# voithru/voice-activity-detection

Hardware: AMD Instinct MI355X
Metric: audio frames/sec (whole node) (higher is better)
Workload: dtype f32 (bf16x6 split operands, f32 accumulate)

## Files before the change

voice_activity_detection_amd/csrc/savad_kernels_f32s.h:

```cpp
#pragma once
#include "savad_kernels_bf16.h"
#include <type_traits>

namespace savad {
#ifdef SAVAD_TIMING
__device__ long long g_savad_wg[1024][4];
#endif
namespace fs {

using bf::bf16x8;
using bf::u32x4;
using bf::ldfrag;
using bf::stfrag;
using bf::FRAG_BYTES;
using bf::slot_row;
using bf::AttnState;
using bf::attn_state_init;
using bf::online_softmax_shifted;

constexpr int SLOT_BYTES = 2 * BLK3_BYTES;
constexpr int NRING3 = 3;
constexpr int ROW_LDS_BYTES = NRING3 * SLOT_BYTES + 9 * D * 4;

struct Tri {
    bf16x8 h, m, l;
};

__device__ __forceinline__ void split1(float a, __bf16& h, __bf16& m, __bf16& l) {
    h = (__bf16)a;
    if (SAVAD_ABLATE & 128) {
        m = l = h;
        return;
    }
    const float r1 = a - (float)h;
    m = (__bf16)r1;
    const float r2 = r1 - (float)m;
    l = (__bf16)r2;
}
__device__ __forceinline__ Tri split8(const float (&v)[8]) {
    Tri t;
#pragma unroll
    for (int e = 0; e < 8; ++e) {
        __bf16 h, m, l;
        split1(v[e], h, m, l);
        t.h[e] = h;
        t.m[e] = m;
        t.l[e] = l;
    }
    return t;
}
__device__ __forceinline__ Tri split_half(const f32x16& v, int j) {
    float t[8];
#pragma unroll
    for (int e = 0; e < 8; ++e) t[e] = v[8 * j + e];
    return split8(t);
}
__device__ __forceinline__ void split_row(const f32x4 (&xg)[16], Tri (&xp)[8]) {
#pragma unroll
    for (int ks = 0; ks < 8; ++ks) {
        float t[8];
#pragma unroll
        for (int e = 0; e < 8; ++e) t[e] = xg[2 * ks + (e >> 2)][e & 3];
        xp[ks] = split8(t);
    }
}
__device__ __forceinline__ Tri ldtri(const char* p ) {
    return Tri{ldfrag(p), ldfrag(p + FRAG_BYTES), ldfrag(p + 2 * FRAG_BYTES)};
}
__device__ __forceinline__ void sttri(char* p, const Tri& t) {
    stfrag(p, t.h);
    stfrag(p + FRAG_BYTES, t.m);
    stfrag(p + 2 * FRAG_BYTES, t.l);
}
__device__ __forceinline__ Tri zero_tri() {
    const bf16x8 z = __builtin_bit_cast(bf16x8, u32x4{0u, 0u, 0u, 0u});
    return Tri{z, z, z};
}

#define SAVAD_MF(a, b, c) __builtin_amdgcn_mfma_f32_32x32x16_bf16((a), (b), (c), 0, 0, 0)
template <bool SWAP>
__device__ __forceinline__ void mfma6x2_lo(f32x16& acc0, f32x16& acc1, const Tri& a0, const Tri& a1, const Tri& b) {
#define SAVAD_MF2(pa, pb)                                                           \
    acc0 = SWAP ? SAVAD_MF(b.pb, a0.pa, acc0) : SAVAD_MF(a0.pa, b.pb, acc0);        \
    acc1 = SWAP ? SAVAD_MF(b.pb, a1.pa, acc1) : SAVAD_MF(a1.pa, b.pb, acc1);
    SAVAD_MF2(h, l) SAVAD_MF2(l, h) SAVAD_MF2(m, m)
}
template <bool SWAP>
__device__ __forceinline__ void mfma6x2_hi(f32x16& acc0, f32x16& acc1, const Tri& a0, const Tri& a1, const Tri& b) {
    SAVAD_MF2(h, m) SAVAD_MF2(m, h) SAVAD_MF2(h, h)
#undef SAVAD_MF2
}
template <bool SWAP>
__device__ __forceinline__ void mfma6x2(f32x16& acc0, f32x16& acc1, const Tri& a0, const Tri& a1, const Tri& b) {
    mfma6x2_lo<SWAP>(acc0, acc1, a0, a1, b);
    mfma6x2_hi<SWAP>(acc0, acc1, a0, a1, b);
}

__device__ __forceinline__ void load_hblock32(f32x16 (&x)[4], const float* hb, int lane) {
#pragma unroll
    for (int nb = 0; nb < 4; ++nb)
#pragma unroll
        for (int g = 0; g < 4; ++g) {
            const f32x4 t = ld4(hb + ((nb * 4 + g) * 64 + lane) * 4);
#pragma unroll
            for (int s = 0; s < 4; ++s) x[nb][4 * g + s] += t[s];
        }
}
__device__ __forceinline__ void request_hblock32(f32x4 (&hr)[16], const float* hb , int lane) {
#define SAVAD_H_LD(i)                                                                                                          \
    asm volatile("global_load_dwordx4 %0, %1, %2 offset:%3" : "+v"(hr[i]) : "v"((unsigned)lane * 16u + 4096u * ((i) / 4)), "s"(hb), \
                 "n"(((i) % 4) * 1024) : "memory")
    SAVAD_H_LD(0); SAVAD_H_LD(1); SAVAD_H_LD(2); SAVAD_H_LD(3); SAVAD_H_LD(4); SAVAD_H_LD(5); SAVAD_H_LD(6); SAVAD_H_LD(7);
    SAVAD_H_LD(8); SAVAD_H_LD(9); SAVAD_H_LD(10); SAVAD_H_LD(11); SAVAD_H_LD(12); SAVAD_H_LD(13); SAVAD_H_LD(14); SAVAD_H_LD(15);
#undef SAVAD_H_LD
}
__device__ __forceinline__ void landed_hblock32(f32x4 (&hr)[16]) {
    asm volatile("" : "+v"(hr[0]), "+v"(hr[1]), "+v"(hr[2]), "+v"(hr[3]), "+v"(hr[4]), "+v"(hr[5]), "+v"(hr[6]), "+v"(hr[7]), "+v"(hr[8]),
                 "+v"(hr[9]), "+v"(hr[10]), "+v"(hr[11]), "+v"(hr[12]), "+v"(hr[13]), "+v"(hr[14]), "+v"(hr[15]));
}
__device__ __forceinline__ void store_hblock32(float* hb, const f32x16 (&x)[4], int lane) {
#pragma unroll
    for (int nb = 0; nb < 4; ++nb)
#pragma unroll
        for (int g = 0; g < 4; ++g) {
            f32x4 t;
#pragma unroll
            for (int s = 0; s < 4; ++s) t[s] = x[nb][4 * g + s];
            st4(hb + ((nb * 4 + g) * 64 + lane) * 4, t);
        }
}

#ifndef SAVAD_PIECE_FENCE
#define SAVAD_PIECE_FENCE 0x6
#endif
struct DmaJob {
    const char* src;
    unsigned ldsb;
};
struct Ring3 {
    static constexpr int PER = 12;
    char* base;
    int w, lane;
    unsigned voff[3];

    __device__ __forceinline__ Ring3(char* smem, int w_, int lane_) : base(smem), w(w_), lane(lane_) {
#pragma unroll
        for (int g = 0; g < 3; ++g) voff[g] = (unsigned)lane_ * 16u + 4096u * g;
    }
    __device__ __forceinline__ char* slot(int t) const { return base + (t % NRING3) * SLOT_BYTES; }
    __device__ __forceinline__ DmaJob job(int t, const char* seg0, const char* seg1) const {
        const unsigned slot0 = __builtin_amdgcn_readfirstlane((unsigned)(size_t)slot(t));
        return DmaJob{((w >> 1) ? seg1 : seg0) + (size_t)(w & 1) * (BLK3_BYTES / 2), slot0 + (unsigned)w * (BLK3_BYTES / 2)};
    }
    template <int I>
    __device__ __forceinline__ void piece(const DmaJob& j) const {
        if (SAVAD_ABLATE & 1) return;
        __builtin_amdgcn_sched_barrier(SAVAD_PIECE_FENCE);
        piece_raw<I>(j);
        __builtin_amdgcn_sched_barrier(SAVAD_PIECE_FENCE);
    }
    template <int I>
    __device__ __forceinline__ void piece_raw(const DmaJob& j) const {
        asm volatile(
            "s_add_u32 m0, %2, %3\n\t"
            "s_nop 0\n\t"
            "global_load_lds_dwordx4 %0, %1 offset:%4"
            :
            : "v"(voff[I / 4]), "s"(j.src), "s"(j.ldsb), "n"((I / 4) * 4096), "n"((I % 4) * 1024)
            : "memory", "scc");
    }
    __device__ __forceinline__ void issue_all(const DmaJob& j) const {
        if (SAVAD_ABLATE & 1) return;
        piece_raw<0>(j); piece_raw<1>(j); piece_raw<2>(j); piece_raw<3>(j); piece_raw<4>(j); piece_raw<5>(j);
        piece_raw<6>(j); piece_raw<7>(j); piece_raw<8>(j); piece_raw<9>(j); piece_raw<10>(j); piece_raw<11>(j);
    }
    template <int NEWER>
    __device__ __forceinline__ void acquire() const {
        if (SAVAD_ABLATE & 2) return;
        __builtin_amdgcn_s_waitcnt(bf::Ring<4>::vmcnt_imm(NEWER * PER));
        asm volatile("" ::: "memory");
        __syncthreads();
    }
};

struct NoMid {
    template <int KS>
    __device__ __forceinline__ void operator()(std::integral_constant<int, KS>) const {}
};
template <bool SWAP, bool DMA, class Mid = NoMid>
__device__ __forceinline__ void gemm_slot(f32x16& acc0, f32x16& acc1, const char* slot, const Tri (&xp)[8], const Ring3& ring,
                                          const DmaJob& job, const Mid& mid = Mid{}) {
    if (SAVAD_ABLATE & 8) {
#pragma unroll
        for (int ks = 0; ks < 8; ++ks) mfma6x2<SWAP>(acc0, acc1, xp[7 - ks], xp[ks ^ 1], xp[ks]);
        return;
    }
    const unsigned a = (unsigned)(size_t)slot + (unsigned)ring.lane * 16u;
    u32x4 f[2][6];
#define SAVAD_G_LD(ks, i) asm volatile("ds_read_b128 %0, %1 offset:%2" : "=v"(f[(ks) & 1][i]) : "v"(a), "n"(((i) / 3) * BLK3_BYTES + (ks) * TFRAG_BYTES + ((i) % 3) * FRAG_BYTES))
#define SAVAD_G_LD6(ks) SAVAD_G_LD(ks, 0); SAVAD_G_LD(ks, 1); SAVAD_G_LD(ks, 2); SAVAD_G_LD(ks, 3); SAVAD_G_LD(ks, 4); SAVAD_G_LD(ks, 5)
#define SAVAD_G_STEP(ks, P0, P1)                                                                                              \
    {                                                                                                                         \
        if constexpr ((ks) + 1 < 8) { SAVAD_G_LD6((ks) + 1); }                                                                \
        asm volatile("s_waitcnt lgkmcnt(%6)"                                                                                  \
                     : "+v"(f[(ks) & 1][0]), "+v"(f[(ks) & 1][1]), "+v"(f[(ks) & 1][2]), "+v"(f[(ks) & 1][3]), "+v"(f[(ks) & 1][4]), \
                       "+v"(f[(ks) & 1][5])                                                                                   \
                     : "n"((ks) + 1 < 8 ? 6 : 0));                                                                            \
        const Tri w0_{__builtin_bit_cast(bf16x8, f[(ks) & 1][0]), __builtin_bit_cast(bf16x8, f[(ks) & 1][1]),                  \
                      __builtin_bit_cast(bf16x8, f[(ks) & 1][2])};                                                            \
        const Tri w1_{__builtin_bit_cast(bf16x8, f[(ks) & 1][3]), __builtin_bit_cast(bf16x8, f[(ks) & 1][4]),                  \
                      __builtin_bit_cast(bf16x8, f[(ks) & 1][5])};                                                            \
        mfma6x2_lo<SWAP>(acc0, acc1, w0_, w1_, xp[ks]);                                                                       \
        if constexpr (DMA && (P1) >= 0) ring.template piece<((P1) >= 0 ? (P1) : 0)>(job);                                     \
        mid(std::integral_constant<int, (ks)>{});                                                                             \
        mfma6x2_hi<SWAP>(acc0, acc1, w0_, w1_, xp[ks]);                                                                       \
        if constexpr (DMA) ring.template piece<P0>(job);                                                                      \
    }
    SAVAD_G_LD6(0);
    SAVAD_G_STEP(0, 1, 0) SAVAD_G_STEP(1, 2, -1) SAVAD_G_STEP(2, 4, 3) SAVAD_G_STEP(3, 5, -1)
    SAVAD_G_STEP(4, 7, 6) SAVAD_G_STEP(5, 8, -1) SAVAD_G_STEP(6, 10, 9) SAVAD_G_STEP(7, 11, -1)
#undef SAVAD_G_STEP
#undef SAVAD_G_LD6
#undef SAVAD_G_LD
}

__global__ void pack_weight_frags3_kernel(const float* __restrict__ W, int N, int K, __bf16* __restrict__ out) {
    const int KS = K / 16;
    const size_t total = (size_t)(N / 32) * KS * 64 * 8;
    for (size_t i = (size_t)blockIdx.x * blockDim.x + threadIdx.x; i < total; i += (size_t)gridDim.x * blockDim.x) {
        const int e = (int)(i & 7);
        const int lane = (int)((i >> 3) & 63);
        const size_t f = i >> 9;
        const int ks = (int)(f % KS);
        const int nblk = (int)(f / KS);
        const int n = lane & 31, h = lane >> 5;
        const int k = 32 * (ks >> 1) + 16 * (ks & 1) + 8 * (e >> 2) + 4 * h + (e & 3);
        __bf16 ph, pm, pl;
        split1(W[(size_t)(32 * nblk + n) * K + k], ph, pm, pl);
        const size_t o = f * 3 * 512 + (size_t)lane * 8 + e;
        out[o] = ph;
        out[o + 512] = pm;
        out[o + 1024] = pl;
    }
}

__global__ void fold_vo_kernel(const float* __restrict__ Wo, const float* __restrict__ Wv, const float* __restrict__ bqkv,
                               float* __restrict__ Wvo, float* __restrict__ bvo) {
    const int n = blockIdx.x, k = threadIdx.x;
    double acc = 0.0, accb = 0.0;
    for (int j = 0; j < D; ++j) {
        const double w = (double)Wo[(size_t)n * D + j];
        acc += w * (double)Wv[(size_t)j * D + k];
        accb += w * (double)bqkv[2 * D + j];
    }
    Wvo[(size_t)n * D + k] = (float)acc;
    if (k == 0) bvo[n] = (float)accb;
}

__global__ void fold_qk_kernel(const float* __restrict__ Wq, const float* __restrict__ Wk, const float* __restrict__ bq, double c,
                               float* __restrict__ Wqt, float* __restrict__ bqt) {
    const int n = blockIdx.x, k = threadIdx.x;
    double acc = 0.0, accb = 0.0;
    for (int o = 0; o < D; ++o) {
        const double w = (double)Wk[(size_t)o * D + n];
        acc += w * (double)Wq[(size_t)o * D + k];
        accb += w * (double)bq[o];
    }
    Wqt[(size_t)n * D + k] = (float)(c * acc);
    if (k == 0) bqt[n] = (float)(c * accb);
}

template <int RB, int HALF, bool DMA, bool SCALE, class Mid = NoMid>
__device__ __forceinline__ void qkv_slot(const char* slot, const Tri (&xp)[8], const float* lb, char* __restrict__ dst, int blk,
                                         const Ring3& ring, const DmaJob& job, float qscale, bool live, const Mid& mid = Mid{}) {
    const int lane = ring.lane, n = lane & 31, h = lane >> 5;
    constexpr int nb0 = 2 * HALF;
    f32x16 acc[2];
    if constexpr (RB < 2) {
#pragma unroll
        for (int i = 0; i < 2; ++i) acc[i] = bias_block(lb + 32 * (nb0 + i), h);
        gemm_slot<false, DMA>(acc[0], acc[1], slot, xp, ring, job, mid);
    } else {
#pragma unroll
        for (int i = 0; i < 2; ++i) {
            const float bv = lb[32 * (nb0 + i) + n];
#pragma unroll
            for (int r = 0; r < 16; ++r) acc[i][r] = bv;
        }
        gemm_slot<true, DMA>(acc[0], acc[1], slot, xp, ring, job, mid);
    }
    if constexpr (SCALE) {
        acc[0] *= qscale;
        acc[1] *= qscale;
    }
    if (!live) return;
#pragma unroll
    for (int i = 0; i < 2; ++i)
#pragma unroll
        for (int j = 0; j < 2; ++j)
            sttri(dst + (size_t)blk * BLK3_BYTES + (2 * (nb0 + i) + j) * TFRAG_BYTES + lane * 16, split_half(acc[i], j));
}
template <int S, bool QKF, bool DMA, class Mid = NoMid>
__device__ __forceinline__ void qkv_image_slot(const char* slot, const Tri (&xp)[8], const float* lbq, char* __restrict__ qf, char* __restrict__ kf,
                                               char* __restrict__ vtf, int blk, const Ring3& ring, const DmaJob& job, float qscale, bool live,
                                               const Mid& mid = Mid{}) {
    constexpr int pos = S >> 1, rb = QKF ? 2 * pos : pos;
    qkv_slot<rb, (S & 1), DMA, (rb == 0 && !QKF)>(slot, xp, lbq + D * pos, rb == 0 ? qf : (rb == 1 ? kf : vtf), blk, ring, job, qscale, live, mid);
}

#ifndef SAVAD_KSTORE
#define SAVAD_KSTORE 2
#endif
__device__ __forceinline__ void store_k_tri(char* kblk , const Tri (&xp)[8], int ks, int lane) {
    sttri(kblk + ks * TFRAG_BYTES + lane * 16, xp[ks]);
}
__device__ __forceinline__ void store_k_burst(char* kblk, const Tri (&xp)[8], int lane, bool live) {
    if (!live) return;
#pragma unroll
    for (int ks = 0; ks < 8; ++ks) store_k_tri(kblk, xp, ks, lane);
}
template <int S>
struct KStoreMid {
    char* kblk;
    const Tri (&xp)[8];
    int lane;
    bool live;
    template <int KS>
    __device__ __forceinline__ void operator()(std::integral_constant<int, KS>) const {
        if constexpr ((KS & 1) && ((SAVAD_KSTORE == 2 && S == 0) || SAVAD_KSTORE == 3)) {
            __builtin_amdgcn_sched_barrier(SAVAD_PIECE_FENCE);
            if (live) {
                if constexpr (SAVAD_KSTORE == 2) {
                    store_k_tri(kblk, xp, KS - 1, lane);
                    store_k_tri(kblk, xp, KS, lane);
                } else {
                    store_k_tri(kblk, xp, 4 * S + (KS >> 1), lane);
                }
            }
            __builtin_amdgcn_sched_barrier(SAVAD_PIECE_FENCE);
        }
    }
};

__device__ __forceinline__ Tri load_x_tri(const float* p, bool valid) {
    f32x4 a = __builtin_nontemporal_load(reinterpret_cast<const f32x4*>(p)), b = __builtin_nontemporal_load(reinterpret_cast<const f32x4*>(p + 8));
    if (!valid) a = b = f32x4{0.f, 0.f, 0.f, 0.f};
    float t[8];
#pragma unroll
    for (int e = 0; e < 4; ++e) {
        t[e] = a[e];
        t[4 + e] = b[e];
    }
    return split8(t);
}

__device__ __forceinline__ void input_gemm_f32s(f32x16 (&h0)[4], const float* xr, bool valid, const char* win, int KS, int lane, int h) {
    constexpr int KSMAX = 8;
    f32x4 xa[KSMAX], xc[KSMAX];
#pragma unroll
    for (int ks = 0; ks < KSMAX; ++ks) {
        const int kc = ks < KS ? ks : KS - 1;
        const float* px = xr + 32 * (kc >> 1) + 16 * (kc & 1) + 4 * h;
        xa[ks] = __builtin_nontemporal_load(reinterpret_cast<const f32x4*>(px));
        xc[ks] = __builtin_nontemporal_load(reinterpret_cast<const f32x4*>(px + 8));
    }
    auto wtri = [&](int nb, int ks) { return ldtri(win + (size_t)(nb * KS + (ks < KS ? ks : KS - 1)) * TFRAG_BYTES + lane * 16); };
    Tri wn[4] = {wtri(0, 0), wtri(1, 0), wtri(2, 0), wtri(3, 0)};
#pragma unroll
    for (int ks = 0; ks < KSMAX; ++ks)
        if (ks < KS) {
            const Tri w0 = wn[0], w1 = wn[1], w2 = wn[2], w3 = wn[3];
            if (ks + 1 < KSMAX) {
#pragma unroll
                for (int nb = 0; nb < 4; ++nb) wn[nb] = wtri(nb, ks + 1);
            }
            float t[8];
#pragma unroll
            for (int e = 0; e < 4; ++e) {
                t[e] = valid ? xa[ks][e] : 0.0f;
                t[4 + e] = valid ? xc[ks][e] : 0.0f;
            }
            const Tri xf = split8(t);
            mfma6x2<false>(h0[0], h0[1], w0, w1, xf);
            mfma6x2<false>(h0[2], h0[3], w2, w3, xf);
        }
    for (int ks = KSMAX; ks < KS; ++ks) {
        const int f0 = 32 * (ks >> 1) + 16 * (ks & 1) + 4 * h;
        const Tri xf = load_x_tri(xr + f0, valid);
#pragma unroll
        for (int nb = 0; nb < 4; nb += 2)
            mfma6x2<false>(h0[nb], h0[nb + 1], ldtri(win + (size_t)(nb * KS + ks) * TFRAG_BYTES + lane * 16),
                           ldtri(win + (size_t)((nb + 1) * KS + ks) * TFRAG_BYTES + lane * 16), xf);
    }
}

template <bool QKF>
__device__ __forceinline__ void input_qkv_f32s(char* smem, const float* __restrict__ x, long xbs, int B, int T, int F, int nblk,
                                               const char* __restrict__ win_frag, const float* __restrict__ bin, const float* __restrict__ pe,
                                               const char* __restrict__ wqkv_frag, const float* __restrict__ bqkv, float* __restrict__ hbuf,
                                               char* __restrict__ qf, char* __restrict__ kf, char* __restrict__ vtf, float qscale) {
    float* lbq = reinterpret_cast<float*>(smem + NRING3 * SLOT_BYTES);
    const int lane = threadIdx.x & 63, m = lane & 31, h = lane >> 5;
    const int w = __builtin_amdgcn_readfirstlane(threadIdx.x >> 6);
    const int blk = blockIdx.x * 4 + w;
    const Ring3 ring(smem, w, lane);
    auto job = [&](int t) { return ring.job(t, wqkv_frag + (size_t)(2 * t) * BLK3_BYTES, wqkv_frag + (size_t)(2 * t + 1) * BLK3_BYTES); };
    SAVAD_STAMP(57);
    ring.issue_all(job(0));
    ring.issue_all(job(1));
    stage_bias(lbq, bqkv, (QKF ? 2 : 3) * D);
    SAVAD_STAMP(58);
    size_t row;
    int t_frame;
    const bool valid = (blk < nblk) && slot_row(B, T, blk, m, row, t_frame);
    if (!valid) {
        row = 0;
        t_frame = 0;
    }
    f32x16 h0[4];
#pragma unroll
    for (int nb = 0; nb < 4; ++nb) {
        h0[nb] = zero16();
        add_bias(h0[nb], bin + 32 * nb, h);
        add_block(h0[nb], pe + (size_t)t_frame * D + 32 * nb, h);
    }
    input_gemm_f32s(h0, x + x_row_offset(row, T, F, xbs), valid, win_frag, F / 16, lane, h);
    SAVAD_STAMP(59);
    const bool live = blk < nblk;
    if (live) store_hblock32(hbuf + (size_t)blk * (32 * D), h0, lane);
    f32x4 xg[16];
    layernorm_regs(h0, xg);
    Tri xp[8];
    split_row(xg, xp);
    SAVAD_STAMP(60);
    const DmaJob none{nullptr, 0u};
    constexpr int NS = QKF ? 4 : 6;
    char* kblk = kf + (size_t)blk * BLK3_BYTES;
#define SAVAD_IQ_STEP(T_, mid)                                                                                                 \
    ring.acquire<((T_) + 1 < NS) ? 1 : 0>();                                                                                   \
    if (QKF && SAVAD_KSTORE == 1 && (T_) == 0) store_k_burst(kblk, xp, lane, live);                                            \
    qkv_image_slot<T_, QKF, ((T_) + 2 < NS)>(ring.slot(T_), xp, lbq, qf, kf, vtf, blk, ring, (T_) + 2 < NS ? job((T_) + 2) : none, qscale, \
                                             live, mid);
    if constexpr (QKF) {
        if (SAVAD_KSTORE == 0) store_k_burst(kblk, xp, lane, live);
        SAVAD_IQ_STEP(0, (KStoreMid<0>{kblk, xp, lane, live})) SAVAD_IQ_STEP(1, (KStoreMid<1>{kblk, xp, lane, live}))
        SAVAD_STAMP(61);
        SAVAD_IQ_STEP(2, NoMid{}) SAVAD_IQ_STEP(3, NoMid{})
        SAVAD_STAMP(63);
    } else {
        SAVAD_IQ_STEP(0, NoMid{}) SAVAD_IQ_STEP(1, NoMid{})
        SAVAD_STAMP(61);
        SAVAD_IQ_STEP(2, NoMid{}) SAVAD_IQ_STEP(3, NoMid{})
        SAVAD_STAMP(62);
        SAVAD_IQ_STEP(4, NoMid{}) SAVAD_IQ_STEP(5, NoMid{})
        SAVAD_STAMP(63);
    }
#undef SAVAD_IQ_STEP
}
__global__ __launch_bounds__(256, 1) void input_qkv_kernel_f32s(const float* __restrict__ x, long xbs, int B, int T, int F, int nblk,
                                                                const char* __restrict__ win_frag, const float* __restrict__ bin,
                                                                const float* __restrict__ pe, const char* __restrict__ wqkv_frag,
                                                                const float* __restrict__ bqkv, float* __restrict__ hbuf,
                                                                char* __restrict__ qf, char* __restrict__ kf, char* __restrict__ vtf,
                                                                float qscale) {
    extern __shared__ __attribute__((aligned(16))) char smem[];
    input_qkv_f32s<true>(smem, x, xbs, B, T, F, nblk, win_frag, bin, pe, wqkv_frag, bqkv, hbuf, qf, kf, vtf, qscale);
}
__global__ __launch_bounds__(256, 1) void input_qkv_kernel_f32s_plain(const float* __restrict__ x, long xbs, int B, int T, int F, int nblk,
                                                                      const char* __restrict__ win_frag, const float* __restrict__ bin,
                                                                      const float* __restrict__ pe, const char* __restrict__ wqkv_frag,
                                                                      const float* __restrict__ bqkv, float* __restrict__ hbuf,
                                                                      char* __restrict__ qf, char* __restrict__ kf, char* __restrict__ vtf,
                                                                      float qscale) {
    extern __shared__ __attribute__((aligned(16))) char smem[];
    input_qkv_f32s<false>(smem, x, xbs, B, T, F, nblk, win_frag, bin, pe, wqkv_frag, bqkv, hbuf, qf, kf, vtf, qscale);
}

typedef __bf16 bf16x2 __attribute__((ext_vector_type(2)));
__device__ __forceinline__ void split_pair(float a0, float a1, unsigned& h, unsigned& m, unsigned& l) {
    __bf16 h0, m0, l0, h1, m1, l1;
    split1(a0, h0, m0, l0);
    split1(a1, h1, m1, l1);
    h = __builtin_bit_cast(unsigned, bf16x2{h0, h1});
    m = __builtin_bit_cast(unsigned, bf16x2{m0, m1});
    l = __builtin_bit_cast(unsigned, bf16x2{l0, l1});
}
__device__ __forceinline__ void settle_reference(f32x16& sc, AttnState& st, bool first ) {
    float mx = sc[0];
#pragma unroll
    for (int r = 1; r < 16; ++r) mx = fmaxf(mx, sc[r]);
    mx = half_max(mx);
    const bool move = (mx > RESCALE_LOG2) || (first && mx < -RESCALE_LOG2);
    if (__any(move)) {
        const float d = move ? mx : 0.0f;
        if (!first) {
            const float alpha = __builtin_amdgcn_exp2f(-d);
            st.l_run *= alpha;
#pragma unroll
            for (int nb = 0; nb < 4; ++nb) st.O[nb] *= alpha;
        }
#pragma unroll
        for (int r = 0; r < 16; ++r) {
            sc[r] -= d;
            st.negm[r] -= d;
        }
    }
}
__device__ __forceinline__ f32x16 qk_tile3(const AttnState& st, const Tri (&qp)[8], const char* kblk, int lane) {
    f32x16 sa = st.negm, sb = zero16();
#pragma unroll
    for (int ks = 0; ks < 8; ++ks) {
        const Tri k = ldtri(kblk + ks * TFRAG_BYTES + lane * 16);
        sa = SAVAD_MF(k.h, qp[ks].l, sa);
        sb = SAVAD_MF(k.l, qp[ks].h, sb);
        sa = SAVAD_MF(k.m, qp[ks].m, sa);
        sb = SAVAD_MF(k.h, qp[ks].m, sb);
        sa = SAVAD_MF(k.m, qp[ks].h, sa);
        sb = SAVAD_MF(k.h, qp[ks].h, sb);
    }
    return sa + sb;
}
template <bool HAVE_NEXT, bool DMA, class MaskNext>
__device__ __forceinline__ void attn_step3(AttnState& st, const Tri (&qp)[8], f32x16& sc, const char* slot, MaskNext mask_next,
                                           const Ring3& ring, const DmaJob& job) {
    const unsigned av = (unsigned)(size_t)slot + (unsigned)ring.lane * 16u, ak = av + BLK3_BYTES;
    f32x16 sa = st.negm, sb = zero16();
    unsigned ph[8], pm[8], pl[8];
    float rs = 0.0f;
    u32x4 fk[3][3];
    u32x4 fv[2][6];
#define SAVAD_A_LDK(ks, i) asm volatile("ds_read_b128 %0, %1 offset:%2" : "=v"(fk[(ks) % 3][i]) : "v"(ak), "n"((ks) * TFRAG_BYTES + (i) * FRAG_BYTES))
#define SAVAD_A_LDK3(ks) SAVAD_A_LDK(ks, 0); SAVAD_A_LDK(ks, 1); SAVAD_A_LDK(ks, 2)
#define SAVAD_A_LDV(g, i) asm volatile("ds_read_b128 %0, %1 offset:%2" : "=v"(fv[(g) & 1][i]) : "v"(av), "n"((((2 * ((g) >> 1) + (i) / 3) * 2 + ((g) & 1)) * 3 + (i) % 3) * FRAG_BYTES))
#define SAVAD_A_LDV6(g) SAVAD_A_LDV(g, 0); SAVAD_A_LDV(g, 1); SAVAD_A_LDV(g, 2); SAVAD_A_LDV(g, 3); SAVAD_A_LDV(g, 4); SAVAD_A_LDV(g, 5)
#define SAVAD_A_SOFT(ks)                                                                                                       \
    {                                                                                                                          \
        const float e0_ = (SAVAD_ABLATE & 4) ? sc[2 * (ks)] : __builtin_amdgcn_exp2f(sc[2 * (ks)]);                            \
        const float e1_ = (SAVAD_ABLATE & 4) ? sc[2 * (ks) + 1] : __builtin_amdgcn_exp2f(sc[2 * (ks) + 1]);                    \
        rs += e0_;                                                                                                             \
        rs += e1_;                                                                                                             \
        split_pair(e0_, e1_, ph[ks], pm[ks], pl[ks]);                                                                          \
    }
#define SAVAD_A_QK(ks)                                                                                                         \
    {                                                                                                                          \
        if constexpr ((ks) + 2 < 8) { SAVAD_A_LDK3((ks) + 2); }                                                                \
        if constexpr ((ks) == 6) { SAVAD_A_LDV6(0); }                                                                          \
        asm volatile("s_waitcnt lgkmcnt(%3)" : "+v"(fk[(ks) % 3][0]), "+v"(fk[(ks) % 3][1]), "+v"(fk[(ks) % 3][2])             \
                     : "n"((ks) + 2 < 8 ? 6 : ((ks) == 6 ? 9 : 6)));                                                           \
        const bf16x8 kh_ = __builtin_bit_cast(bf16x8, fk[(ks) % 3][0]), km_ = __builtin_bit_cast(bf16x8, fk[(ks) % 3][1]),     \
                     kl_ = __builtin_bit_cast(bf16x8, fk[(ks) % 3][2]);                                                        \
        sa = SAVAD_MF(kh_, qp[ks].l, sa);                                                                                      \
        sb = SAVAD_MF(kl_, qp[ks].h, sb);                                                                                      \
        sa = SAVAD_MF(km_, qp[ks].m, sa);                                                                                      \
        sb = SAVAD_MF(kh_, qp[ks].m, sb);                                                                                      \
        sa = SAVAD_MF(km_, qp[ks].h, sa);                                                                                      \
        sb = SAVAD_MF(kh_, qp[ks].h, sb);                                                                                      \
        SAVAD_A_SOFT(ks)                                                                                                       \
    }
    if constexpr (HAVE_NEXT) {
        SAVAD_A_LDK3(0);
        SAVAD_A_LDK3(1);
        SAVAD_A_QK(0) SAVAD_A_QK(1) SAVAD_A_QK(2) SAVAD_A_QK(3) SAVAD_A_QK(4) SAVAD_A_QK(5) SAVAD_A_QK(6) SAVAD_A_QK(7)
    } else {
        SAVAD_A_LDV6(0);
        SAVAD_A_SOFT(0) SAVAD_A_SOFT(1) SAVAD_A_SOFT(2) SAVAD_A_SOFT(3) SAVAD_A_SOFT(4) SAVAD_A_SOFT(5) SAVAD_A_SOFT(6) SAVAD_A_SOFT(7)
    }
#undef SAVAD_A_QK
#undef SAVAD_A_SOFT
#undef SAVAD_A_LDK3
#undef SAVAD_A_LDK
    st.l_run += rs;
    const Tri p0{__builtin_bit_cast(bf16x8, u32x4{ph[0], ph[1], ph[2], ph[3]}), __builtin_bit_cast(bf16x8, u32x4{pm[0], pm[1], pm[2], pm[3]}),
                 __builtin_bit_cast(bf16x8, u32x4{pl[0], pl[1], pl[2], pl[3]})};
    const Tri p1{__builtin_bit_cast(bf16x8, u32x4{ph[4], ph[5], ph[6], ph[7]}), __builtin_bit_cast(bf16x8, u32x4{pm[4], pm[5], pm[6], pm[7]}),
                 __builtin_bit_cast(bf16x8, u32x4{pl[4], pl[5], pl[6], pl[7]})};
#define SAVAD_A_PV(g, PJ)                                                                                                      \
    {                                                                                                                          \
        if constexpr ((g) + 1 < 4) { SAVAD_A_LDV6((g) + 1); }                                                                  \
        asm volatile("s_waitcnt lgkmcnt(%6)"                                                                                   \
                     : "+v"(fv[(g) & 1][0]), "+v"(fv[(g) & 1][1]), "+v"(fv[(g) & 1][2]), "+v"(fv[(g) & 1][3]), "+v"(fv[(g) & 1][4]), \
                       "+v"(fv[(g) & 1][5])                                                                                    \
                     : "n"((g) + 1 < 4 ? 6 : 0));                                                                              \
        const Tri v0_{__builtin_bit_cast(bf16x8, fv[(g) & 1][0]), __builtin_bit_cast(bf16x8, fv[(g) & 1][1]),                   \
                      __builtin_bit_cast(bf16x8, fv[(g) & 1][2])};                                                             \
        const Tri v1_{__builtin_bit_cast(bf16x8, fv[(g) & 1][3]), __builtin_bit_cast(bf16x8, fv[(g) & 1][4]),                   \
                      __builtin_bit_cast(bf16x8, fv[(g) & 1][5])};                                                             \
        mfma6x2<false>(st.O[2 * ((g) >> 1)], st.O[2 * ((g) >> 1) + 1], v0_, v1_, PJ);                                          \
        if constexpr (DMA) {                                                                                                   \
            ring.template piece<3 * (g)>(job);                                                                                 \
            ring.template piece<3 * (g) + 1>(job);                                                                             \
            ring.template piece<3 * (g) + 2>(job);                                                                             \
        }                                                                                                                      \
    }
    SAVAD_A_PV(0, p0) SAVAD_A_PV(1, p1)
    if constexpr (HAVE_NEXT) {
        sc = sa + sb;
        mask_next(sc);
    }
    SAVAD_A_PV(2, p0) SAVAD_A_PV(3, p1)
#undef SAVAD_A_PV
#undef SAVAD_A_LDV6
#undef SAVAD_A_LDV
    if constexpr (HAVE_NEXT) settle_reference(sc, st, false);
}
template <class Mask>
__device__ __forceinline__ void attn_tile3_global(AttnState& st, const Tri (&qp)[8], const char* kblk, const char* vtblk, Mask mask, int lane) {
    f32x16 sa = st.negm, sb = zero16();
#pragma unroll
    for (int ks = 0; ks < 8; ++ks) {
        const Tri k = ldtri(kblk + ks * TFRAG_BYTES + lane * 16);
        sa = SAVAD_MF(k.h, qp[ks].l, sa);
        sb = SAVAD_MF(k.l, qp[ks].h, sb);
        sa = SAVAD_MF(k.m, qp[ks].m, sa);
        sb = SAVAD_MF(k.h, qp[ks].m, sb);
        sa = SAVAD_MF(k.m, qp[ks].h, sa);
        sb = SAVAD_MF(k.h, qp[ks].h, sb);
    }
    f32x16 sc = sa + sb;
    mask(sc);
    online_softmax_shifted(sc, st, true);
    const Tri p0 = split_half(sc, 0), p1 = split_half(sc, 1);
#pragma unroll
    for (int nbd = 0; nbd < 4; nbd += 2) {
        mfma6x2<false>(st.O[nbd], st.O[nbd + 1], ldtri(vtblk + ((nbd * 2 + 0) * TFRAG_BYTES) + lane * 16),
                       ldtri(vtblk + (((nbd + 1) * 2 + 0) * TFRAG_BYTES) + lane * 16), p0);
        mfma6x2<false>(st.O[nbd], st.O[nbd + 1], ldtri(vtblk + ((nbd * 2 + 1) * TFRAG_BYTES) + lane * 16),
                       ldtri(vtblk + (((nbd + 1) * 2 + 1) * TFRAG_BYTES) + lane * 16), p1);
    }
}

struct RowArgs3 {
    int B, T, nblk;
    float* hbuf;
    const char* wo_frag;
    const float* bo;
    const char* w1_frag;
    const float* b1;
    const char* w2_frag;
    const float* b2;
    const char* wn_frag;
    const float* wc;
    const float* bn;
    char *qf, *kf, *vtf;
    float* out;
    float qscale;
};
__device__ __forceinline__ const char* row_seg(const RowArgs3& A, int t, int sgm, bool folded) {
    if (!folded) {
        if (t < 2) return A.wo_frag + (size_t)(2 * t + sgm) * BLK3_BYTES;
        t -= 2;
    }
    if (t < 16) {
        const int c = t >> 2, r = t & 3;
        return r < 2 ? A.w1_frag + (size_t)(4 * c + 2 * r + sgm) * BLK3_BYTES
                     : A.w2_frag + (size_t)((2 * (r - 2) + sgm) * 32 + 8 * c) * TFRAG_BYTES;
    }
    return A.wn_frag + (size_t)(2 * (t - 16) + sgm) * BLK3_BYTES;
}

template <bool LAST, bool FOLDED>
struct RowBiases {
    BiasPiece pieces[4];
    BiasRegs<4> regs;
    float bc;
    float* lbn;
    __device__ __forceinline__ RowBiases(const RowArgs3& A, char* smem) {
        float* lbo = reinterpret_cast<float*>(smem + NRING3 * SLOT_BYTES);
        float* lb1 = lbo + D;
        float* lb2 = lb1 + DFF;
        lbn = lb2 + D;
        pieces[0] = BiasPiece{lbo, A.bo, D};
        pieces[1] = BiasPiece{lb1, A.b1, DFF};
        pieces[2] = BiasPiece{lb2, A.b2, D};
        pieces[3] = BiasPiece{lbn, LAST ? A.wc : A.bn, (LAST || FOLDED) ? 2 * D : 3 * D};
        regs = request_bias_pieces(pieces);
        bc = LAST ? A.bn[threadIdx.x & 1] : 0.0f;
    }
    __device__ __forceinline__ void commit() const {
        commit_bias_pieces(pieces, regs);
        if (LAST && threadIdx.x < 2) lbn[2 * D + threadIdx.x] = bc;
    }
};

template <bool LAST, bool FOLDED>
__device__ __forceinline__ void row_stage_f32s(const RowArgs3& A, char* smem, Tri (&xp)[8], const f32x16 (&hc)[4], f32x4 (&hr)[16], int blk,
                                               bool live, const Ring3& ring, int base) {
    float* lbo = reinterpret_cast<float*>(smem + NRING3 * SLOT_BYTES);
    float* lb1 = lbo + D;
    float* lb2 = lb1 + DFF;
    float* lbn = lb2 + D;
    const int lane = ring.lane, m = lane & 31, h = lane >> 5;
    constexpr int OFF = FOLDED ? 0 : 2;
    constexpr int NSLOT = OFF + (LAST ? 16 : FOLDED ? 20 : 22);
    auto job = [&](int t) { return ring.job(base + t, row_seg(A, t, 0, FOLDED), row_seg(A, t, 1, FOLDED)); };
    const DmaJob none{nullptr, 0u};
#define SAVAD_ROW_GEMM(T_, acc0, acc1, operand)                                                                               \
    if ((T_) < 8) SAVAD_STAMP(24 + 3 * (T_));                                                                                 \
    if constexpr (!(FOLDED && (T_) == 0)) ring.acquire<((T_) + 1 < NSLOT) ? 1 : 0>();    \
    if ((T_) < 8) SAVAD_STAMP(25 + 3 * (T_));                                                                                 \
    gemm_slot<false, ((T_) + 2 < NSLOT)>(acc0, acc1, ring.slot(base + (T_)), operand, ring, (T_) + 2 < NSLOT ? job((T_) + 2) : none); \
    if ((T_) < 8) SAVAD_STAMP(26 + 3 * (T_));
    float* hb = A.hbuf + (size_t)blk * (32 * D);
    f32x16 h1[4];
    if constexpr (FOLDED) {
        ring.acquire<1>();
        landed_hblock32(hr);
#pragma unroll
        for (int nb = 0; nb < 4; ++nb) {
            h1[nb] = bias_block(lbo + 32 * nb, h) + hc[nb];
#pragma unroll
            for (int r = 0; r < 16; ++r) h1[nb][r] += hr[4 * nb + (r >> 2)][r & 3];
        }
    } else {
        ring.issue_all(job(0));
        ring.issue_all(job(1));
        ring.acquire<1>();
        f32x16 hres[4];
#pragma unroll
        for (int nb = 0; nb < 4; ++nb) hres[nb] = zero16();
        if (live) load_hblock32(hres, hb, lane);
#pragma unroll
        for (int nb = 0; nb < 4; ++nb) h1[nb] = bias_block(lbo + 32 * nb, h);
        gemm_slot<false, true>(h1[0], h1[1], ring.slot(base), xp, ring, job(2));
        SAVAD_ROW_GEMM(1, h1[2], h1[3], xp)
#pragma unroll
        for (int nb = 0; nb < 4; ++nb) h1[nb] += hres[nb];
    }
    SAVAD_STAMP(5);
    f32x4 xg[16];
    layernorm_regs(h1, xg);
    split_row(xg, xp);
    SAVAD_STAMP(6);
    f32x16(&o)[4] = h1;
#pragma unroll
    for (int nb = 0; nb < 4; ++nb) o[nb] += bias_block(lb2 + 32 * nb, h);
#define SAVAD_ROW_FFN(ch)                                                                                                     \
    {                                                                                                                         \
        f32x16 a[4];                                                                                                          \
        _Pragma("unroll") for (int nbl = 0; nbl < 4; ++nbl) a[nbl] = bias_block(lb1 + 128 * (ch) + 32 * nbl, h);              \
        SAVAD_ROW_GEMM(OFF + 4 * (ch), a[0], a[1], xp)                                                                        \
        SAVAD_ROW_GEMM(OFF + 1 + 4 * (ch), a[2], a[3], xp)                                                                          \
        if ((ch) == 0) SAVAD_STAMP(20);                                                                                       \
        Tri ap[8];                                                                                                            \
        _Pragma("unroll") for (int nbl = 0; nbl < 4; ++nbl) {                                                                 \
            _Pragma("unroll") for (int r = 0; r < 16; ++r) a[nbl][r] = fmaxf(a[nbl][r], 0.0f);                                \
            ap[2 * nbl] = split_half(a[nbl], 0);                                                                              \
            ap[2 * nbl + 1] = split_half(a[nbl], 1);                                                                          \
        }                                                                                                                     \
        if ((ch) == 0) SAVAD_STAMP(21);                                                                                       \
        SAVAD_ROW_GEMM(OFF + 2 + 4 * (ch), o[0], o[1], ap)                                                                    \
        SAVAD_ROW_GEMM(OFF + 3 + 4 * (ch), o[2], o[3], ap)                                                                          \
        SAVAD_STAMP(7 + (ch));                                                                                                \
    }
    SAVAD_ROW_FFN(0) SAVAD_ROW_FFN(1) SAVAD_ROW_FFN(2) SAVAD_ROW_FFN(3)
#undef SAVAD_ROW_FFN
#undef SAVAD_ROW_GEMM
    if (!LAST && live) store_hblock32(hb, o, lane);
    layernorm_regs(o, xg);
    if constexpr (!LAST) {
        split_row(xg, xp);
        SAVAD_STAMP(11);
        char* kblk = A.kf + (size_t)blk * BLK3_BYTES;
#define SAVAD_ROW_QKV(S_, mid)                                                                                                \
    ring.acquire<(OFF + 16 + (S_) + 1 < NSLOT) ? 1 : 0>();                                                                    \
    if (FOLDED && SAVAD_KSTORE == 1 && (S_) == 0) store_k_burst(kblk, xp, lane, live);                                        \
    qkv_image_slot<S_, FOLDED, (OFF + 16 + (S_) + 2 < NSLOT)>(ring.slot(base + OFF + 16 + (S_)), xp, lbn, A.qf, A.kf, A.vtf, blk, ring, \
                                                              OFF + 16 + (S_) + 2 < NSLOT ? job(OFF + 16 + (S_) + 2) : none, A.qscale, live, mid); \
    SAVAD_STAMP(12 + (S_));
        if constexpr (FOLDED) {
            if (SAVAD_KSTORE == 0) store_k_burst(kblk, xp, lane, live);
            SAVAD_ROW_QKV(0, (KStoreMid<0>{kblk, xp, lane, live})) SAVAD_ROW_QKV(1, (KStoreMid<1>{kblk, xp, lane, live}))
            SAVAD_ROW_QKV(2, NoMid{}) SAVAD_ROW_QKV(3, NoMid{})
        } else {
            SAVAD_ROW_QKV(0, NoMid{}) SAVAD_ROW_QKV(1, NoMid{}) SAVAD_ROW_QKV(2, NoMid{}) SAVAD_ROW_QKV(3, NoMid{}) SAVAD_ROW_QKV(4, NoMid{})
            SAVAD_ROW_QKV(5, NoMid{})
        }
#undef SAVAD_ROW_QKV
    } else {
        const f32x2 lp = classify_rows(xg, lbn, lbn + 2 * D, h);
        size_t row;
        int t_frame;
        const bool valid = live && (blk < A.nblk) && slot_row(A.B, A.T, blk, m, row, t_frame);
        if (h == 0 && valid) *reinterpret_cast<f32x2*>(A.out + row * 2) = lp;
    }
}

template <bool LAST, bool PACKED>
__global__ __launch_bounds__(256, 1) void attention_row_kernel_f32s(const char* __restrict__ qf, const char* __restrict__ kf,
                                                                    const char* __restrict__ vtf, int NG, RowArgs3 A) {
    extern __shared__ __attribute__((aligned(16))) char smem[];
    const int B = A.B, T = A.T;
    const int lane = threadIdx.x & 63, m = lane & 31, h = lane >> 5;
    const int w = __builtin_amdgcn_readfirstlane(threadIdx.x >> 6);
    const Ring3 ring(smem, w, lane);
    AttnState st;
    attn_state_init(st);
    Tri qp[8];
    int blk_q, base = 0;
    bool active, qvalid;
    f32x4 hr[16];
#pragma unroll
    for (int i = 0; i < 16; ++i) hr[i] = f32x4{0.f, 0.f, 0.f, 0.f};
    SAVAD_STAMP(0);
#ifdef SAVAD_TIMING
    if (threadIdx.x == 0 && blockIdx.x < 1024) {
        g_savad_wg[blockIdx.x][0] = __builtin_readcyclecounter();
        g_savad_wg[blockIdx.x][2] = __builtin_amdgcn_s_memrealtime();
    }
#endif
    const RowBiases<LAST, !PACKED> biases(A, smem);
    if constexpr (PACKED) {
        biases.commit();
        blk_q = blockIdx.x * 4 + w;
        active = blk_q < A.nblk;
        const int G = 32 / T;
        qvalid = active && (m < G * T) && (blk_q * G + m / T < B);
        if (active) {
#pragma unroll
            for (int ks = 0; ks < 8; ++ks) qp[ks] = ldtri(qf + (size_t)blk_q * BLK3_BYTES + ks * TFRAG_BYTES + lane * 16);
            bool keyok[16];
#pragma unroll
            for (int r = 0; r < 16; ++r) keyok[r] = packed_key_ok(B, T, blk_q, m, acc_row(r, h));
            auto mask = [&](f32x16& sc) {
#pragma unroll
                for (int r = 0; r < 16; ++r) sc[r] = keyok[r] ? sc[r] : NEG_BIG;
            };
            attn_tile3_global(st, qp, kf + (size_t)blk_q * BLK3_BYTES, vtf + (size_t)blk_q * BLK3_BYTES, mask, lane);
        }
    } else {
        const int QB = (T + 31) / 32;
        int b, g;
        if (!xcd_balanced_map(B, NG, b, g)) return;
        const int qb0 = (g * QB) / NG, qb1 = ((g + 1) * QB) / NG;
        const int qb = qb0 + w;
        active = qb < qb1;
        blk_q = b * QB + (active ? qb : qb0);
        qvalid = active && 32 * qb + m < T;
        base = QB;
        auto job = [&](int u) {
            if (u < QB) {
                const size_t kb = (size_t)b * QB;
                const int uv = u < 0 ? 0 : u, uk = u + 1 < QB ? u + 1 : QB - 1;
                return ring.job(u + 3, vtf + (kb + uv) * BLK3_BYTES, kf + (kb + uk) * BLK3_BYTES);
            }
            return ring.job(u, row_seg(A, u - QB, 0, true), row_seg(A, u - QB, 1, true));
        };
        ring.issue_all(job(-1));
#pragma unroll
        for (int ks = 0; ks < 8; ++ks) qp[ks] = ldtri(qf + (size_t)blk_q * BLK3_BYTES + ks * TFRAG_BYTES + lane * 16);
        ring.issue_all(job(0));
        ring.issue_all(job(1));
        biases.commit();
        const int lim = T - 32 * (QB - 1) - 4 * h;
        auto no_mask = [](f32x16&) {};
        auto tail_mask = [&](f32x16& sc) {
            if (32 * QB > T) {
                asm volatile("" ::: "memory");
#pragma unroll
                for (int r = 0; r < 16; ++r) sc[r] = (acc_row(r, 0) < lim) ? sc[r] : NEG_BIG;
            }
        };
        ring.acquire<2>();
        SAVAD_STAMP(1);
        if (active) {
            f32x16 sc = qk_tile3(st, qp, ring.slot(2) + BLK3_BYTES, lane);
            settle_reference(sc, st, true);
            SAVAD_STAMP(2);
#pragma unroll 1
            for (int jt = 0; jt + 2 < QB; ++jt) {
                ring.acquire<1>();
                attn_step3<true, true>(st, qp, sc, ring.slot(jt), no_mask, ring, job(jt + 2));
            }
            ring.acquire<1>();
            attn_step3<true, true>(st, qp, sc, ring.slot(QB - 2), tail_mask, ring, job(QB));
            ring.acquire<1>();
            request_hblock32(hr, A.hbuf + (size_t)blk_q * (32 * D), lane);
            attn_step3<false, true>(st, qp, sc, ring.slot(QB - 1), no_mask, ring, job(QB + 1));
            SAVAD_STAMP(3);
        } else {
#pragma unroll 1
            for (int jt = 0; jt < QB; ++jt) {
                ring.acquire<1>();
                ring.issue_all(job(jt + 2));
            }
        }
    }
    Tri xp[8];
    {
        const float inv = qvalid ? 1.0f / half_sum(st.l_run) : 0.0f;
#pragma unroll
        for (int nbd = 0; nbd < 4; ++nbd) {
#pragma unroll
            for (int r = 0; r < 16; ++r) st.O[nbd][r] = qvalid ? st.O[nbd][r] * inv : 0.0f;
            if constexpr (PACKED) {
                xp[2 * nbd] = split_half(st.O[nbd], 0);
                xp[2 * nbd + 1] = split_half(st.O[nbd], 1);
            }
        }
    }
    SAVAD_STAMP(4);
    row_stage_f32s<LAST, !PACKED>(A, smem, xp, st.O, hr, blk_q, active, ring, base);
    SAVAD_STAMP(18);
#ifdef SAVAD_TIMING
    if (threadIdx.x == 0 && blockIdx.x < 1024) {
        g_savad_wg[blockIdx.x][1] = __builtin_readcyclecounter();
        g_savad_wg[blockIdx.x][3] = __builtin_amdgcn_s_memrealtime();
    }
#endif
}

struct PackedF32sLayer {
    const char *wqkv, *wo, *w1, *w2;
};
struct PackedF32sModel {
    PackedF32sLayer layer[PACKED_F32S_MAX_LAYERS];
    const char* win;
    const float* bin;
    const float* pe;
    const float* bias;
    const float *wc, *bc;
    int L;
};
inline constexpr int packed_f32s_lds_bytes(int L) { return NRING3 * SLOT_BYTES + (L * LBIAS + 2 * D + 4) * 4; }
__device__ __forceinline__ const char* packed_seg(const PackedF32sLayer& Lw, int i, int sgm) {
// ... 523 lines not shown
```

Before: 87.01 million.

## Trim m0 setup in DMA pieces, pin Q in AGPRs, vectorize split

Skips redundant m0 writes and s_nop in most global_load_lds pieces when no mid-callback can clobber m0. Replaces the score MFMA chain with inline asm that keeps Q fragments in AGPRs and uses a zero-accumulator first MFMA plus explicit wait states. Vectorizes the bf16 triple split with packed conversions. Separates the K-store scheduling form for the input and fused paths, with the input path now defaulting to form 3. Hand-managed hazards (nops, m0 reuse) risk correctness if the schedule shifts.

```diff
diff --git a/voice_activity_detection_amd/csrc/savad_kernels_f32s.h b/voice_activity_detection_amd/csrc/savad_kernels_f32s.h
--- a/voice_activity_detection_amd/csrc/savad_kernels_f32s.h
+++ b/voice_activity_detection_amd/csrc/savad_kernels_f32s.h
@@ -152,22 +152,25 @@
         const unsigned slot0 = __builtin_amdgcn_readfirstlane((unsigned)(size_t)slot(t));
         return DmaJob{((w >> 1) ? seg1 : seg0) + (size_t)(w & 1) * (BLK3_BYTES / 2), slot0 + (unsigned)w * (BLK3_BYTES / 2)};
     }
-    template <int I>
+    template <int I, bool M0_EACH = true>
     __device__ __forceinline__ void piece(const DmaJob& j) const {
         if (SAVAD_ABLATE & 1) return;
         __builtin_amdgcn_sched_barrier(SAVAD_PIECE_FENCE);
-        piece_raw<I>(j);
+        piece_raw<I, M0_EACH>(j);
         __builtin_amdgcn_sched_barrier(SAVAD_PIECE_FENCE);
     }
-    template <int I>
+    template <int I, bool M0_EACH = true>
     __device__ __forceinline__ void piece_raw(const DmaJob& j) const {
-        asm volatile(
-            "s_add_u32 m0, %2, %3\n\t"
-            "s_nop 0\n\t"
-            "global_load_lds_dwordx4 %0, %1 offset:%4"
-            :
-            : "v"(voff[I / 4]), "s"(j.src), "s"(j.ldsb), "n"((I / 4) * 4096), "n"((I % 4) * 1024)
-            : "memory", "scc");
+        if constexpr (M0_EACH || I % 4 == 0)
+            asm volatile(
+                "s_add_u32 m0, %2, %3\n\t"
+                "s_nop 0\n\t"
+                "global_load_lds_dwordx4 %0, %1 offset:%4"
+                :
+                : "v"(voff[I / 4]), "s"(j.src), "s"(j.ldsb), "n"((I / 4) * 4096), "n"((I % 4) * 1024)
+                : "memory", "scc");
+        else
+            asm volatile("global_load_lds_dwordx4 %0, %1 offset:%2" : : "v"(voff[I / 4]), "s"(j.src), "n"((I % 4) * 1024) : "memory");
     }
     __device__ __forceinline__ void issue_all(const DmaJob& j) const {
         if (SAVAD_ABLATE & 1) return;
@@ -197,6 +200,7 @@
     }
     const unsigned a = (unsigned)(size_t)slot + (unsigned)ring.lane * 16u;
     u32x4 f[2][6];
+    constexpr bool M0E = !std::is_same<Mid, NoMid>::value;
 #define SAVAD_G_LD(ks, i) asm volatile("ds_read_b128 %0, %1 offset:%2" : "=v"(f[(ks) & 1][i]) : "v"(a), "n"(((i) / 3) * BLK3_BYTES + (ks) * TFRAG_BYTES + ((i) % 3) * FRAG_BYTES))
 #define SAVAD_G_LD6(ks) SAVAD_G_LD(ks, 0); SAVAD_G_LD(ks, 1); SAVAD_G_LD(ks, 2); SAVAD_G_LD(ks, 3); SAVAD_G_LD(ks, 4); SAVAD_G_LD(ks, 5)
 #define SAVAD_G_STEP(ks, P0, P1)                                                                                              \
@@ -211,10 +215,10 @@
         const Tri w1_{__builtin_bit_cast(bf16x8, f[(ks) & 1][3]), __builtin_bit_cast(bf16x8, f[(ks) & 1][4]),                  \
                       __builtin_bit_cast(bf16x8, f[(ks) & 1][5])};                                                            \
         mfma6x2_lo<SWAP>(acc0, acc1, w0_, w1_, xp[ks]);                                                                       \
-        if constexpr (DMA && (P1) >= 0) ring.template piece<((P1) >= 0 ? (P1) : 0)>(job);                                     \
+        if constexpr (DMA && (P1) >= 0) ring.template piece<((P1) >= 0 ? (P1) : 0), M0E>(job);                                     \
         mid(std::integral_constant<int, (ks)>{});                                                                             \
         mfma6x2_hi<SWAP>(acc0, acc1, w0_, w1_, xp[ks]);                                                                       \
-        if constexpr (DMA) ring.template piece<P0>(job);                                                                      \
+        if constexpr (DMA) ring.template piece<P0, M0E>(job);                                                                 \
     }
     SAVAD_G_LD6(0);
     SAVAD_G_STEP(0, 1, 0) SAVAD_G_STEP(1, 2, -1) SAVAD_G_STEP(2, 4, 3) SAVAD_G_STEP(3, 5, -1)
@@ -308,8 +312,12 @@
     qkv_slot<rb, (S & 1), DMA, (rb == 0 && !QKF)>(slot, xp, lbq + D * pos, rb == 0 ? qf : (rb == 1 ? kf : vtf), blk, ring, job, qscale, live, mid);
 }
 
-#ifndef SAVAD_KSTORE
-#define SAVAD_KSTORE 2
+#ifdef SAVAD_KSTORE
+#define SAVAD_KSTORE_INPUT SAVAD_KSTORE
+#define SAVAD_KSTORE_FUSED SAVAD_KSTORE
+#else
+#define SAVAD_KSTORE_INPUT 3
+#define SAVAD_KSTORE_FUSED 2
 #endif
 __device__ __forceinline__ void store_k_tri(char* kblk , const Tri (&xp)[8], int ks, int lane) {
     sttri(kblk + ks * TFRAG_BYTES + lane * 16, xp[ks]);
@@ -319,7 +327,7 @@
 #pragma unroll
     for (int ks = 0; ks < 8; ++ks) store_k_tri(kblk, xp, ks, lane);
 }
-template <int S>
+template <int S, int FORM>
 struct KStoreMid {
     char* kblk;
     const Tri (&xp)[8];
@@ -327,10 +335,10 @@
     bool live;
     template <int KS>
     __device__ __forceinline__ void operator()(std::integral_constant<int, KS>) const {
-        if constexpr ((KS & 1) && ((SAVAD_KSTORE == 2 && S == 0) || SAVAD_KSTORE == 3)) {
+        if constexpr ((KS & 1) && ((FORM == 2 && S == 0) || FORM == 3)) {
             __builtin_amdgcn_sched_barrier(SAVAD_PIECE_FENCE);
             if (live) {
-                if constexpr (SAVAD_KSTORE == 2) {
+                if constexpr (FORM == 2) {
                     store_k_tri(kblk, xp, KS - 1, lane);
                     store_k_tri(kblk, xp, KS, lane);
                 } else {
@@ -438,12 +446,13 @@
     char* kblk = kf + (size_t)blk * BLK3_BYTES;
 #define SAVAD_IQ_STEP(T_, mid)                                                                                                 \
     ring.acquire<((T_) + 1 < NS) ? 1 : 0>();                                                                                   \
-    if (QKF && SAVAD_KSTORE == 1 && (T_) == 0) store_k_burst(kblk, xp, lane, live);                                            \
+    if (QKF && SAVAD_KSTORE_INPUT == 1 && (T_) == 0) store_k_burst(kblk, xp, lane, live);                                            \
     qkv_image_slot<T_, QKF, ((T_) + 2 < NS)>(ring.slot(T_), xp, lbq, qf, kf, vtf, blk, ring, (T_) + 2 < NS ? job((T_) + 2) : none, qscale, \
                                              live, mid);
     if constexpr (QKF) {
-        if (SAVAD_KSTORE == 0) store_k_burst(kblk, xp, lane, live);
-        SAVAD_IQ_STEP(0, (KStoreMid<0>{kblk, xp, lane, live})) SAVAD_IQ_STEP(1, (KStoreMid<1>{kblk, xp, lane, live}))
+        if (SAVAD_KSTORE_INPUT == 0) store_k_burst(kblk, xp, lane, live);
+        SAVAD_IQ_STEP(0, (KStoreMid<0, SAVAD_KSTORE_INPUT>{kblk, xp, lane, live}))
+        SAVAD_IQ_STEP(1, (KStoreMid<1, SAVAD_KSTORE_INPUT>{kblk, xp, lane, live}))
         SAVAD_STAMP(61);
         SAVAD_IQ_STEP(2, NoMid{}) SAVAD_IQ_STEP(3, NoMid{})
         SAVAD_STAMP(63);
@@ -477,13 +486,21 @@
 }
 
 typedef __bf16 bf16x2 __attribute__((ext_vector_type(2)));
+__device__ __forceinline__ float sub1(float a, float b) {
+    float r;
+    asm("v_sub_f32 %0, %1, %2" : "=v"(r) : "v"(a), "v"(b));
+    return r;
+}
 __device__ __forceinline__ void split_pair(float a0, float a1, unsigned& h, unsigned& m, unsigned& l) {
-    __bf16 h0, m0, l0, h1, m1, l1;
-    split1(a0, h0, m0, l0);
-    split1(a1, h1, m1, l1);
-    h = __builtin_bit_cast(unsigned, bf16x2{h0, h1});
-    m = __builtin_bit_cast(unsigned, bf16x2{m0, m1});
-    l = __builtin_bit_cast(unsigned, bf16x2{l0, l1});
+    h = __builtin_bit_cast(unsigned, __builtin_convertvector(f32x2{a0, a1}, bf16x2));
+    if (SAVAD_ABLATE & 128) {
+        m = l = h;
+        return;
+    }
+    const float r0 = sub1(a0, __builtin_bit_cast(float, h << 16)), r1 = sub1(a1, __builtin_bit_cast(float, h & 0xffff0000u));
+    m = __builtin_bit_cast(unsigned, __builtin_convertvector(f32x2{r0, r1}, bf16x2));
+    const float s0 = sub1(r0, __builtin_bit_cast(float, m << 16)), s1 = sub1(r1, __builtin_bit_cast(float, m & 0xffff0000u));
+    l = __builtin_bit_cast(unsigned, __builtin_convertvector(f32x2{s0, s1}, bf16x2));
 }
 __device__ __forceinline__ void settle_reference(f32x16& sc, AttnState& st, bool first ) {
     float mx = sc[0];
@@ -506,25 +523,51 @@
         }
     }
 }
-__device__ __forceinline__ f32x16 qk_tile3(const AttnState& st, const Tri (&qp)[8], const char* kblk, int lane) {
-    f32x16 sa = st.negm, sb = zero16();
-#pragma unroll
-    for (int ks = 0; ks < 8; ++ks) {
-        const Tri k = ldtri(kblk + ks * TFRAG_BYTES + lane * 16);
-        sa = SAVAD_MF(k.h, qp[ks].l, sa);
-        sb = SAVAD_MF(k.l, qp[ks].h, sb);
-        sa = SAVAD_MF(k.m, qp[ks].m, sa);
-        sb = SAVAD_MF(k.h, qp[ks].m, sb);
-        sa = SAVAD_MF(k.m, qp[ks].h, sa);
-        sb = SAVAD_MF(k.h, qp[ks].h, sb);
-    }
+#define SAVAD_MFV_FIRST(d, a, b, c) asm volatile("s_nop 1\n\tv_mfma_f32_32x32x16_bf16 %0, %1, %2, %3" : "=&v"(d) : "v"(a), "a"(b), "v"(c))
+#define SAVAD_MFV_ZERO(d, a, b) asm volatile("v_mfma_f32_32x32x16_bf16 %0, %1, %2, 0" : "=&v"(d) : "v"(a), "a"(b))
+#define SAVAD_MFV(d, a, b) asm volatile("v_mfma_f32_32x32x16_bf16 %0, %1, %2, %0" : "+v"(d) : "v"(a), "a"(b))
+#define SAVAD_SCORE_STEP(ks, sa, sb, kh, km, kl, qp, negm)                                                                     \
+    if constexpr ((ks) == 0) {                                                                                                 \
+        SAVAD_MFV_FIRST(sa, kh, (qp)[ks].l, negm);                                                                             \
+        SAVAD_MFV_ZERO(sb, kl, (qp)[ks].h);                                                                                    \
+    } else {                                                                                                                   \
+        SAVAD_MFV(sa, kh, (qp)[ks].l);                                                                                         \
+        SAVAD_MFV(sb, kl, (qp)[ks].h);                                                                                         \
+    }                                                                                                                          \
+    SAVAD_MFV(sa, km, (qp)[ks].m);                                                                                             \
+    SAVAD_MFV(sb, kh, (qp)[ks].m);                                                                                             \
+    SAVAD_MFV(sa, km, (qp)[ks].h);                                                                                             \
+    SAVAD_MFV(sb, kh, (qp)[ks].h);
+__device__ __forceinline__ void score_q_agpr(Tri (&qp)[8]) {
+#pragma unroll
+    for (int ks = 0; ks < 8; ++ks) asm volatile("" : "+a"(qp[ks].h), "+a"(qp[ks].m), "+a"(qp[ks].l));
+}
+template <bool PAD>
+__device__ __forceinline__ void score_landed(f32x16& sa, f32x16& sb) {
+    if constexpr (PAD)
+        asm volatile("s_nop 11" : "+v"(sa), "+v"(sb));
+    else
+        asm volatile("" : "+v"(sa), "+v"(sb));
+}
+__device__ __forceinline__ f32x16 qk_tile3(const AttnState& st, Tri (&qp)[8], const char* kblk, int lane) {
+    f32x16 sa, sb;
+    score_q_agpr(qp);
+#define SAVAD_QK0(ks)                                                                                                          \
+    {                                                                                                                          \
+        const Tri k_ = ldtri(kblk + (ks) * TFRAG_BYTES + lane * 16);                                                           \
+        SAVAD_SCORE_STEP(ks, sa, sb, k_.h, k_.m, k_.l, qp, st.negm)                                                            \
+    }
+    SAVAD_QK0(0) SAVAD_QK0(1) SAVAD_QK0(2) SAVAD_QK0(3) SAVAD_QK0(4) SAVAD_QK0(5) SAVAD_QK0(6) SAVAD_QK0(7)
+#undef SAVAD_QK0
+    score_landed<true>(sa, sb);
     return sa + sb;
 }
 template <bool HAVE_NEXT, bool DMA, class MaskNext>
-__device__ __forceinline__ void attn_step3(AttnState& st, const Tri (&qp)[8], f32x16& sc, const char* slot, MaskNext mask_next,
+__device__ __forceinline__ void attn_step3(AttnState& st, Tri (&qp)[8], f32x16& sc, const char* slot, MaskNext mask_next,
                                            const Ring3& ring, const DmaJob& job) {
+    static_assert(DMA || !HAVE_NEXT, "the scores' wait states count on the DMA pieces of region B (score_landed)");
     const unsigned av = (unsigned)(size_t)slot + (unsigned)ring.lane * 16u, ak = av + BLK3_BYTES;
-    f32x16 sa = st.negm, sb = zero16();
+    f32x16 sa, sb;
     unsigned ph[8], pm[8], pl[8];
     float rs = 0.0f;
     u32x4 fk[3][3];
@@ -549,15 +592,11 @@
                      : "n"((ks) + 2 < 8 ? 6 : ((ks) == 6 ? 9 : 6)));                                                           \
         const bf16x8 kh_ = __builtin_bit_cast(bf16x8, fk[(ks) % 3][0]), km_ = __builtin_bit_cast(bf16x8, fk[(ks) % 3][1]),     \
                      kl_ = __builtin_bit_cast(bf16x8, fk[(ks) % 3][2]);                                                        \
-        sa = SAVAD_MF(kh_, qp[ks].l, sa);                                                                                      \
-        sb = SAVAD_MF(kl_, qp[ks].h, sb);                                                                                      \
-        sa = SAVAD_MF(km_, qp[ks].m, sa);                                                                                      \
-        sb = SAVAD_MF(kh_, qp[ks].m, sb);                                                                                      \
-        sa = SAVAD_MF(km_, qp[ks].h, sa);                                                                                      \
-        sb = SAVAD_MF(kh_, qp[ks].h, sb);                                                                                      \
+        SAVAD_SCORE_STEP(ks, sa, sb, kh_, km_, kl_, qp, st.negm)                                                               \
         SAVAD_A_SOFT(ks)                                                                                                       \
     }
     if constexpr (HAVE_NEXT) {
+        score_q_agpr(qp);
         SAVAD_A_LDK3(0);
         SAVAD_A_LDK3(1);
         SAVAD_A_QK(0) SAVAD_A_QK(1) SAVAD_A_QK(2) SAVAD_A_QK(3) SAVAD_A_QK(4) SAVAD_A_QK(5) SAVAD_A_QK(6) SAVAD_A_QK(7)
@@ -587,13 +626,14 @@
                       __builtin_bit_cast(bf16x8, fv[(g) & 1][5])};                                                             \
         mfma6x2<false>(st.O[2 * ((g) >> 1)], st.O[2 * ((g) >> 1) + 1], v0_, v1_, PJ);                                          \
         if constexpr (DMA) {                                                                                                   \
-            ring.template piece<3 * (g)>(job);                                                                                 \
-            ring.template piece<3 * (g) + 1>(job);                                                                             \
-            ring.template piece<3 * (g) + 2>(job);                                                                             \
+            ring.template piece<3 * (g), (g) == 2>(job);                 \
+            ring.template piece<3 * (g) + 1, false>(job);                                                                      \
+            ring.template piece<3 * (g) + 2, false>(job);                                                                      \
         }                                                                                                                      \
     }
     SAVAD_A_PV(0, p0) SAVAD_A_PV(1, p1)
     if constexpr (HAVE_NEXT) {
+        score_landed<false>(sa, sb);
         sc = sa + sb;
         mask_next(sc);
     }
@@ -763,13 +803,14 @@
         char* kblk = A.kf + (size_t)blk * BLK3_BYTES;
 #define SAVAD_ROW_QKV(S_, mid)                                                                                                \
     ring.acquire<(OFF + 16 + (S_) + 1 < NSLOT) ? 1 : 0>();                                                                    \
-    if (FOLDED && SAVAD_KSTORE == 1 && (S_) == 0) store_k_burst(kblk, xp, lane, live);                                        \
+    if (FOLDED && SAVAD_KSTORE_FUSED == 1 && (S_) == 0) store_k_burst(kblk, xp, lane, live);                                        \
     qkv_image_slot<S_, FOLDED, (OFF + 16 + (S_) + 2 < NSLOT)>(ring.slot(base + OFF + 16 + (S_)), xp, lbn, A.qf, A.kf, A.vtf, blk, ring, \
                                                               OFF + 16 + (S_) + 2 < NSLOT ? job(OFF + 16 + (S_) + 2) : none, A.qscale, live, mid); \
     SAVAD_STAMP(12 + (S_));
         if constexpr (FOLDED) {
-            if (SAVAD_KSTORE == 0) store_k_burst(kblk, xp, lane, live);
-            SAVAD_ROW_QKV(0, (KStoreMid<0>{kblk, xp, lane, live})) SAVAD_ROW_QKV(1, (KStoreMid<1>{kblk, xp, lane, live}))
+            if (SAVAD_KSTORE_FUSED == 0) store_k_burst(kblk, xp, lane, live);
+            SAVAD_ROW_QKV(0, (KStoreMid<0, SAVAD_KSTORE_FUSED>{kblk, xp, lane, live}))
+            SAVAD_ROW_QKV(1, (KStoreMid<1, SAVAD_KSTORE_FUSED>{kblk, xp, lane, live}))
             SAVAD_ROW_QKV(2, NoMid{}) SAVAD_ROW_QKV(3, NoMid{})
         } else {
             SAVAD_ROW_QKV(0, NoMid{}) SAVAD_ROW_QKV(1, NoMid{}) SAVAD_ROW_QKV(2, NoMid{}) SAVAD_ROW_QKV(3, NoMid{}) SAVAD_ROW_QKV(4, NoMid{})
```

Result: no change. 87.70 million, median of 4 (+0.8%).
